# envoyproxy/ai-gateway

Hardware: AMD Instinct MI355X
Metric: req/sec (whole node) + p50 added latency, OpenAI chat/completions 4k-token body (higher is better)
Workload: dtype bf16; 1 GPU; model=aigw standalone: OpenAI /v1/chat/completions -> mock upstream (examples/basic), global_batch=128, seq_len=4096, parallelism=dp1, front=fast, cpu_affinity=numa node 0 (128 cpus)

## Files before the change

csrc/aigw_fast_module.cpp:

```cpp

#include <pybind11/pybind11.h>
#include <pybind11/stl.h>

#include <cstdint>
#include <stdexcept>
#include <string>
#include <vector>

#include "fastpath.h"

namespace py = pybind11;
using namespace aigw_fast;

namespace aigw_fast {

GpuAdmissionDirect* admission_create(const long long* htab_keys,
                                     const int32_t* htab_rank, int htab_n,
                                     size_t max_bytes, int max_req, int device);
bool admission_count(GpuAdmissionDirect* a, const char* bytes, size_t n,
                     const int64_t* offsets, int n_req, int32_t* counts_out);
void admission_destroy(GpuAdmissionDirect* a);
bool admission_init_cache(GpuAdmissionDirect* a, const uint16_t* emb, int vocab,
                          const uint16_t* proj, int dim, long long capacity,
                          float threshold, int pending_cap, bool fp8);
// ... 243 lines not shown
          "swap_routes",
          [](FastServer& s, py::list route_specs) {
            std::vector<FastRoute> routes;
            for (auto item : route_specs) {
              py::dict rd = item.cast<py::dict>();
              FastRoute r;
              r.name = rd["name"].cast<std::string>();
              r.model_match = rd["model_match"].cast<std::string>();
              r.retries = rd["retries"].cast<int>();
              r.has_costs = rd["has_costs"].cast<bool>();
              r.eligible = rd["eligible"].cast<bool>();
              for (auto b : rd["backends"].cast<py::list>()) {
                py::dict d = b.cast<py::dict>();
                FastBackend be;
                be.name = d["name"].cast<std::string>();
                be.host = d["host"].cast<std::string>();
                be.port = d["port"].cast<uint16_t>();
                if (d.contains("bearer")) be.bearer = d["bearer"].cast<std::string>();
                if (d.contains("api_key_file"))
                  be.api_key_file = d["api_key_file"].cast<std::string>();
                if (d.contains("model_override"))
                  be.model_override = d["model_override"].cast<std::string>();
                if (d.contains("weight")) be.weight = d["weight"].cast<double>();
                if (d.contains("priority")) be.priority = d["priority"].cast<int>();
                if (d.contains("timeout_s")) be.timeout_s = d["timeout_s"].cast<double>();
                if (d.contains("azure")) be.azure = d["azure"].cast<bool>();
                if (d.contains("azure_api_version"))
                  be.azure_api_version = d["azure_api_version"].cast<std::string>();
                r.backends.push_back(std::move(be));
              }
              routes.push_back(std::move(r));
            }
            s.swap_routes(std::move(routes));
          },
          "hot-swap the route table (in-flight requests keep the old one)")
      .def("drain", &FastServer::drain, py::arg("drain_s"),
           py::call_guard<py::gil_scoped_release>())
      .def("enable_gpu", &FastServer::enable_gpu, py::arg("socket_path"),
           py::arg("window_us") = 100, py::arg("max_batch") = 256)
      .def(
          "enable_gpu_direct",
          [](FastServer& s, py::buffer htab_keys, py::buffer htab_rank,
             int max_batch, size_t max_batch_bytes, int max_req, int device) {
            py::buffer_info ki = htab_keys.request();
            py::buffer_info ri = htab_rank.request();
            if (ki.itemsize != 8 || ri.itemsize != 4)
              throw std::runtime_error(
                  "htab_keys must be int64, htab_rank int32");
            if (ki.size != ri.size)
              throw std::runtime_error("htab arrays must have equal length");
            s.enable_gpu_direct(static_cast<const long long*>(ki.ptr),
                                static_cast<const int32_t*>(ri.ptr),
                                (int)ki.size, max_batch, max_batch_bytes,
                                max_req, device);
          },
          py::arg("htab_keys"), py::arg("htab_rank"),
          py::arg("max_batch") = 1024,
          py::arg("max_batch_bytes") = (size_t)48 * 1024 * 1024,
          py::arg("max_req") = 4096, py::arg("device") = 0)
      .def(
          "enable_gpu_direct_cache",
          [](FastServer& s, py::buffer emb, py::buffer proj, int dim,
             long long capacity, float threshold, bool fp8) {
            py::buffer_info ei = emb.request();
            py::buffer_info pi = proj.request();
            if (ei.itemsize != 2 || pi.itemsize != 2)
              throw std::runtime_error("emb/proj must be bf16 (uint16 view)");
            int vocab = (int)(ei.size / dim);
            if ((long long)vocab * dim != ei.size || pi.size != (long long)dim * dim)
              throw std::runtime_error("emb/proj shape mismatch");
            if (!s.enable_gpu_direct_cache(
                    static_cast<const uint16_t*>(ei.ptr), vocab,
                    static_cast<const uint16_t*>(pi.ptr), dim, capacity,
                    threshold, fp8))
              throw std::runtime_error("native cache init failed");
          },
          py::arg("emb"), py::arg("proj"), py::arg("dim") = 384,
          py::arg("capacity") = 65536, py::arg("threshold") = 0.92,
          py::arg("fp8") = false)
      .def("start", &FastServer::start, py::arg("host"), py::arg("port"),
           py::call_guard<py::gil_scoped_release>())
      .def("stop", &FastServer::stop, py::call_guard<py::gil_scoped_release>())
      .def("gpu_direct_stats", &FastServer::gpu_direct_stats)
      .def("rl_collect_deltas", &FastServer::rl_collect_deltas)
      .def("rl_apply_remote", &FastServer::rl_apply_remote)
      .def("rl_local_spent", &FastServer::rl_local_spent)
      .def("stats", [](const FastServer& s) {
        const ServerStats& st = s.stats();
        py::dict d;
        d["requests"] = st.requests.load();
        d["responses_2xx"] = st.responses_2xx.load();
        d["responses_4xx"] = st.responses_4xx.load();
        d["responses_5xx"] = st.responses_5xx.load();
        d["local_429"] = st.local_429.load();
        d["fallback"] = st.fallback.load();
        d["retries"] = st.retries.load();
        d["gpu_tokens"] = st.gpu_tokens.load();
        d["cache_hits"] = st.cache_hits.load();
        d["cache_misses"] = st.cache_misses.load();
        d["input_tokens"] = st.input_tokens.load();
        d["output_tokens"] = st.output_tokens.load();
        d["total_tokens"] = st.total_tokens.load();
        d["bytes_in"] = st.bytes_in.load();
        d["bytes_out"] = st.bytes_out.load();
        d["active_connections"] = st.active_connections.load();
        py::list hist;
        for (int i = 0; i < 32; ++i) hist.append(st.latency_us_log2[i].load());
        d["latency_us_log2"] = hist;
        return d;
      });
}
```

csrc/fastpath.cpp:

```cpp

#include "fastpath.h"

#include <arpa/inet.h>
#include <errno.h>
#include <fcntl.h>
#include <netdb.h>
#include <netinet/in.h>
#include <netinet/tcp.h>
#include <string.h>
#include <sys/socket.h>
#include <sys/time.h>
#include <sys/types.h>
#include <sys/un.h>
#include <unistd.h>

#include <algorithm>
#include <chrono>
#include <cmath>
#include <random>

#include "msgpack_mini.h"
#include "native_core.h"

namespace aigw_fast {
// ... 51 lines not shown
  struct msghdr msg;
  memset(&msg, 0, sizeof(msg));
  msg.msg_iov = iov;
  msg.msg_iovlen = 2;
  while (sent < total) {
    ssize_t w = ::sendmsg(fd, &msg, MSG_NOSIGNAL);
    if (w < 0) {
      if (errno == EINTR) continue;
      return false;
    }
    sent += (size_t)w;
    size_t skip = (size_t)w;
    while (msg.msg_iovlen > 0 && skip >= msg.msg_iov[0].iov_len) {
      skip -= msg.msg_iov[0].iov_len;
      ++msg.msg_iov;
      --msg.msg_iovlen;
    }
    if (msg.msg_iovlen > 0) {
      msg.msg_iov[0].iov_base = (char*)msg.msg_iov[0].iov_base + skip;
      msg.msg_iov[0].iov_len -= skip;
    }
  }
  return true;
}

ssize_t read_some(int fd, char* p, size_t cap) {
  for (;;) {
    ssize_t r = ::recv(fd, p, cap, 0);
    if (r < 0 && errno == EINTR) continue;
    return r;
  }
}

int tcp_connect(const std::string& host, uint16_t port, double timeout_s) {
  struct sockaddr_in addr;
  memset(&addr, 0, sizeof(addr));
  addr.sin_family = AF_INET;
  addr.sin_port = htons(port);
  if (inet_pton(AF_INET, host.c_str(), &addr.sin_addr) != 1) {
    struct addrinfo hints, *res = nullptr;
    memset(&hints, 0, sizeof(hints));
    hints.ai_family = AF_INET;
    hints.ai_socktype = SOCK_STREAM;
    if (getaddrinfo(host.c_str(), nullptr, &hints, &res) != 0 || !res) return -1;
    addr.sin_addr = ((struct sockaddr_in*)res->ai_addr)->sin_addr;
    freeaddrinfo(res);
  }
  int fd = ::socket(AF_INET, SOCK_STREAM, 0);
  if (fd < 0) return -1;
  set_timeout(fd, timeout_s);
  if (::connect(fd, (struct sockaddr*)&addr, sizeof(addr)) != 0) {
    ::close(fd);
    return -1;
  }
  set_nodelay(fd);
  return fd;
}

std::string lower(std::string s) {
  for (auto& c : s) c = (char)tolower((unsigned char)c);
  return s;
}

struct Header {
  std::string name;
  std::string value;
};

struct HttpHead {
  std::string method, path;
  int status = 0;
  std::vector<Header> headers;
  size_t head_len = 0;

  const std::string* get(const char* name) const {
    for (const auto& h : headers)
      if (h.name == name) return &h.value;
    return nullptr;
  }
};

constexpr size_t kMaxHead = 64 * 1024;
constexpr size_t kMaxBody = 64 * 1024 * 1024;

bool parse_head(const std::string& buf, size_t head_end, bool is_request, HttpHead* out) {
  out->head_len = head_end + 4;
  size_t line_end = buf.find("\r\n");
  if (line_end == std::string::npos || line_end > head_end) return false;
  const std::string first = buf.substr(0, line_end);
  if (is_request) {
    size_t sp1 = first.find(' ');
    if (sp1 == std::string::npos) return false;
    size_t sp2 = first.find(' ', sp1 + 1);
    if (sp2 == std::string::npos) return false;
    out->method = first.substr(0, sp1);
    out->path = first.substr(sp1 + 1, sp2 - sp1 - 1);
  } else {
    if (first.compare(0, 7, "HTTP/1.") != 0) return false;
    size_t sp = first.find(' ');
    if (sp == std::string::npos) return false;
    out->status = atoi(first.c_str() + sp + 1);
  }
  size_t pos = line_end + 2;
  while (pos < head_end) {
    size_t eol = buf.find("\r\n", pos);
    if (eol == std::string::npos || eol > head_end) eol = head_end;
    size_t colon = buf.find(':', pos);
    if (colon != std::string::npos && colon < eol) {
      Header h;
      h.name = lower(buf.substr(pos, colon - pos));
      size_t vs = colon + 1;
      while (vs < eol && (buf[vs] == ' ' || buf[vs] == '\t')) ++vs;
      size_t ve = eol;
      while (ve > vs && (buf[ve - 1] == ' ' || buf[ve - 1] == '\t')) --ve;
      while (!h.name.empty() && (h.name.back() == ' ' || h.name.back() == '\t'))
        h.name.pop_back();
      h.value = buf.substr(vs, ve - vs);
      out->headers.push_back(std::move(h));
    }
    pos = eol + 2;
  }
  return true;
}


enum class Framing { kLength, kChunked, kClose, kNone };

Framing response_framing(const HttpHead& h, int64_t* length) {
  const std::string* te = h.get("transfer-encoding");
  if (te && lower(*te).find("chunked") != std::string::npos) return Framing::kChunked;
  if (h.status == 204 || h.status == 304 || (h.status >= 100 && h.status < 200)) {
    *length = 0;
    return Framing::kLength;
  }
  const std::string* cl = h.get("content-length");
  if (cl) {
    *length = atoll(cl->c_str());
    return Framing::kLength;
  }
  return Framing::kClose;
}

class ChunkedParser {
 public:
  bool done() const { return state_ == State::kDone; }
  bool error() const { return state_ == State::kError; }

  template <class F>
  void feed(const char* p, size_t n, F&& payload) {
    size_t i = 0;
    while (i < n && state_ != State::kDone && state_ != State::kError) {
      switch (state_) {
        case State::kSize: {
          char c = p[i++];
          line_.push_back(c);
          if (line_.size() > 256) { state_ = State::kError; break; }
          if (c == '\n') {
            size_t semi = line_.find(';');
            std::string hex = line_.substr(0, semi);
            remaining_ = strtoll(hex.c_str(), nullptr, 16);
            line_.clear();
            if (remaining_ < 0) state_ = State::kError;
            else if (remaining_ == 0) state_ = State::kTrailer;
            else state_ = State::kData;
          }
          break;
// ... 307 lines not shown
    std::vector<std::shared_ptr<Waiter>> all;
    {
      std::lock_guard<std::mutex> lk(qmu_);
      all.insert(all.end(), q_waiters_.begin(), q_waiters_.end());
      q_waiters_.clear();
      q_texts_.clear();
    }
    {
      std::lock_guard<std::mutex> lk(pmu_);
      for (auto& kv : pending_)
        all.insert(all.end(), kv.second.begin(), kv.second.end());
      pending_.clear();
    }
    for (auto& w : all) {
      std::lock_guard<std::mutex> lk(w->m);
      w->done = true;
      w->cv.notify_all();
    }
  }

  int fd_ = -1;
  int window_us_ = 100;
  int max_batch_ = 256;
  std::atomic<bool> stopping_{false};
  std::atomic<uint64_t> next_id_{1};
  std::mutex qmu_;
  std::condition_variable qcv_;
  std::vector<std::string> q_texts_;
  std::vector<std::shared_ptr<GpuAdmissionClient::Waiter>> q_waiters_;
  std::mutex pmu_;
  std::map<uint64_t, std::vector<std::shared_ptr<Waiter>>> pending_;
  std::thread batcher_, reader_;
};



GpuAdmissionDirect* admission_create(const long long* htab_keys,
                                     const int32_t* htab_rank, int htab_n,
                                     size_t max_bytes, int max_req, int device);
bool admission_count(GpuAdmissionDirect* a, const char* bytes, size_t n,
                     const int64_t* offsets, int n_req, int32_t* counts_out);
void admission_destroy(GpuAdmissionDirect* a);
bool admission_init_cache(GpuAdmissionDirect* a, const uint16_t* emb, int vocab,
                          const uint16_t* proj, int dim, long long capacity,
                          float threshold, int pending_cap, bool fp8);
bool admission_count_lookup(GpuAdmissionDirect* a, const char* bytes, size_t n,
                            const int64_t* offsets, int n_req,
                            int32_t* counts_out, const int32_t* pending_slots,
                            int32_t* rows_out, float* scores_out);
long long admission_cache_insert(GpuAdmissionDirect* a, int pending_slot);
bool admission_submit(GpuAdmissionDirect* a, int set, const char* bytes,
                      size_t n, const int64_t* offsets, int n_req,
                      const int32_t* pending_slots);
bool admission_wait(GpuAdmissionDirect* a, int set, int n_req,
                    int32_t* counts_out, int32_t* rows_out, float* scores_out);
char* admission_staging(GpuAdmissionDirect* a, int set);

class DirectGpuBatcher {
 public:
  bool start(const long long* htab_keys, const int32_t* htab_rank, int htab_n,
             int max_batch, size_t max_bytes, int max_req, int device) {
    adm_ = admission_create(htab_keys, htab_rank, htab_n, max_bytes, max_req,
                            device);
    if (adm_ == nullptr) return false;
    max_batch_ = std::min(max_batch, max_req);
    max_bytes_ = max_bytes;
    worker_ = std::thread([this] { loop(); });
    return true;
  }

  void stop() {
    stopping_ = true;
    {
      std::lock_guard<std::mutex> lk(mu_);
      cv_.notify_all();
    }
    if (worker_.joinable()) worker_.join();
    if (adm_ != nullptr) admission_destroy(adm_), adm_ = nullptr;
    fail_all();
  }

  ~DirectGpuBatcher() { stop(); }

  int64_t count_text(const std::string& text) {
    CacheLookup cl = count_lookup_text(text);
    cache_release_slot(cl.slot);
    return cl.tokens;
  }

  struct Waiter2 {
    std::mutex m;
    std::condition_variable cv;
    bool done = false;
    int64_t count = 0;
    int32_t row = -1;
    float score = 0.f;
    int32_t slot = -1;
  };

  struct CacheLookup {
    int64_t tokens = 0;
    int32_t row = -1;
    float score = 0.f;
    int32_t slot = -1;
  };

  std::shared_ptr<Waiter2> enqueue(const std::string& text) {
    if (stopping_) return nullptr;
    auto w = std::make_shared<Waiter2>();
    {
      std::lock_guard<std::mutex> lk(mu_);
      q_texts_.push_back(text);
      q_waiters_.push_back(w);
      cv_.notify_one();
    }
    return w;
  }

  CacheLookup collect(const std::shared_ptr<Waiter2>& w) {
    CacheLookup out;
    if (w == nullptr) return out;
    std::unique_lock<std::mutex> lk(w->m);
    w->cv.wait_for(lk, std::chrono::seconds(30), [&] { return w->done; });
    out.tokens = w->count;
    out.row = w->row;
    out.score = w->score;
    out.slot = w->slot;
    return out;
  }

  CacheLookup count_lookup_text(const std::string& text) {
    return collect(enqueue(text));
  }

  bool init_cache(const uint16_t* emb, int vocab, const uint16_t* proj,
                  int dim, long long capacity, float threshold, bool fp8) {
    if (adm_ == nullptr) return false;
    const int pending_cap = 4096;
    if (!admission_init_cache(adm_, emb, vocab, proj, dim, capacity, threshold,
                              pending_cap, fp8))
      return false;
    {
      std::lock_guard<std::mutex> lk(slot_mu_);
      free_slots_.resize(pending_cap);
      for (int i = 0; i < pending_cap; ++i) free_slots_[i] = pending_cap - 1 - i;
    }
    cache_on_ = true;
    return true;
  }

  bool cache_on() const { return cache_on_; }

  long long cache_insert_slot(int slot) {
    long long row;
    {
      std::lock_guard<std::mutex> lk(insert_mu_);
      row = admission_cache_insert(adm_, slot);
    }
    cache_release_slot(slot);
    return row;
  }

  void cache_release_slot(int slot) {
    if (slot < 0) return;
    std::lock_guard<std::mutex> lk(slot_mu_);
    free_slots_.push_back(slot);
  }


 private:
  struct InFlight {
    std::vector<std::shared_ptr<Waiter2>> waiters;
    std::vector<int32_t> slots;
    int64_t t0 = 0;
    bool valid = false;
  };

  void finish_set(int s) {
    InFlight& fl = inflight_[s];
    if (!fl.valid) return;
    int n = (int)fl.waiters.size();
    std::vector<int32_t> counts((size_t)n, 0);
    std::vector<int32_t> rows((size_t)n, -1);
    std::vector<float> scores((size_t)n, 0.f);
    bool want_cache = cache_on_.load();
    int64_t w0 = now_us();
    if (!admission_wait(adm_, s, n, counts.data(),
                        want_cache ? rows.data() : nullptr,
                        want_cache ? scores.data() : nullptr))
      stats_errors++;
    int64_t w1 = now_us();
    stats_wait_us += (uint64_t)(w1 - w0);
    int64_t bt = w1 - fl.t0;
    stats_batches++;
    stats_texts += (uint64_t)n;
    stats_time_us += (uint64_t)bt;
    uint64_t prev = stats_max_us.load();
    while ((uint64_t)bt > prev &&
           !stats_max_us.compare_exchange_weak(prev, (uint64_t)bt)) {}
    for (int i = 0; i < n; ++i) {
      auto& w = fl.waiters[i];
      std::lock_guard<std::mutex> lk(w->m);
      w->count = counts[i];
      w->row = rows[i];
      w->score = scores[i];
      w->slot = fl.slots[i];
      w->done = true;
      w->cv.notify_all();
    }
    stats_fulfill_us += (uint64_t)(now_us() - w1);
    fl.waiters.clear();
    fl.slots.clear();
    fl.valid = false;
  }

  void loop() {
    std::vector<int64_t> offs;
    int next_set = 0;
    while (!stopping_) {
      std::vector<std::string> texts;
      std::vector<std::shared_ptr<Waiter2>> waiters;
      {
        std::unique_lock<std::mutex> lk(mu_);
        if (q_texts_.empty()) {
          int other = 1 - next_set;
          if (inflight_[other].valid) {
            lk.unlock();
            finish_set(other);
            continue;
          }
          cv_.wait(lk, [&] { return stopping_ || !q_texts_.empty(); });
          if (stopping_) break;
        }
        size_t take = 0, bytes = 0;
        while (take < q_texts_.size() && (int)take < max_batch_ &&
               bytes + q_texts_[take].size() <= max_bytes_)
          bytes += q_texts_[take++].size();
        if (take == 0) take = 1;
        texts.assign(q_texts_.begin(), q_texts_.begin() + take);
        waiters.assign(q_waiters_.begin(), q_waiters_.begin() + take);
        q_texts_.erase(q_texts_.begin(), q_texts_.begin() + take);
        q_waiters_.erase(q_waiters_.begin(), q_waiters_.begin() + take);
      }
      finish_set(next_set);
      int64_t p0 = now_us();
      char* stage = admission_staging(adm_, next_set);
      size_t used = 0;
      offs.clear();
      for (auto& t : texts) {
        offs.push_back((int64_t)used);
        size_t room = max_bytes_ - used;
        size_t take_n = std::min(t.size(), room);
        memcpy(stage + used, t.data(), take_n);
        used += take_n;
      }
      size_t nt = texts.size();
      std::vector<int32_t> slots((size_t)nt, -1);
      if (cache_on_) {
        std::lock_guard<std::mutex> lk(slot_mu_);
        for (size_t i = 0; i < nt && !free_slots_.empty(); ++i) {
          slots[i] = free_slots_.back();
          free_slots_.pop_back();
        }
      }
      stats_pack_us += (uint64_t)(now_us() - p0);
      int64_t s0 = now_us();
      bool ok = used > 0 &&
                admission_submit(adm_, next_set, nullptr, used,
                                 offs.data(), (int)nt,
                                 cache_on_ ? slots.data() : nullptr);
      stats_submit_us += (uint64_t)(now_us() - s0);
      if (!ok) {
        if (used > 0) stats_errors++;
        for (size_t i = 0; i < nt; ++i) {
          auto& w = waiters[i];
          std::lock_guard<std::mutex> lk(w->m);
          w->slot = slots[i];
          w->done = true;
          w->cv.notify_all();
        }
        continue;
      }
      InFlight& fl = inflight_[next_set];
      fl.waiters = std::move(waiters);
      fl.slots = std::move(slots);
      fl.t0 = now_us();
      fl.valid = true;
      finish_set(1 - next_set);
      next_set ^= 1;
    }
    finish_set(0);
    finish_set(1);
  }

  void fail_all() {
    std::vector<std::shared_ptr<Waiter2>> all;
    {
      std::lock_guard<std::mutex> lk(mu_);
      all = std::move(q_waiters_);
      q_waiters_.clear();
      q_texts_.clear();
    }
    for (auto& w : all) {
      std::lock_guard<std::mutex> lk(w->m);
      w->done = true;
      w->cv.notify_all();
    }
  }

  GpuAdmissionDirect* adm_ = nullptr;
  std::atomic<bool> cache_on_{false};
  std::mutex slot_mu_;
  std::vector<int32_t> free_slots_;
  std::mutex insert_mu_;

 public:
  std::atomic<uint64_t> stats_batches{0};
  std::atomic<uint64_t> stats_texts{0};
  std::atomic<uint64_t> stats_time_us{0};
  std::atomic<uint64_t> stats_max_us{0};
  std::atomic<uint64_t> stats_errors{0};
  std::atomic<uint64_t> stats_pack_us{0};
  std::atomic<uint64_t> stats_submit_us{0};
  std::atomic<uint64_t> stats_wait_us{0};
  std::atomic<uint64_t> stats_fulfill_us{0};

 private:
  int max_batch_ = 1024;
  size_t max_bytes_ = 0;
  std::atomic<bool> stopping_{false};
  std::mutex mu_;
  std::condition_variable cv_;
  std::vector<std::string> q_texts_;
  std::vector<std::shared_ptr<Waiter2>> q_waiters_;
  InFlight inflight_[2];
  std::thread worker_;
};



namespace {

bool banned_upstream_header(const std::string& name) {
  static const char* kBanned[] = {
      "host", "content-length", "content-type", "connection", "keep-alive",
      "proxy-authenticate", "proxy-authorization", "te", "trailer",
      "transfer-encoding", "upgrade", "expect", "accept-encoding",
      "authorization"};
  for (const char* b : kBanned)
    if (name == b) return true;
  if (name.compare(0, 8, "x-ai-eg-") == 0) return true;
  if (name.compare(0, 7, "x-aigw-") == 0) return true;
  return false;
}

}

class ConnHandler {
 public:
  ConnHandler(FastServer* srv, int fd) : srv_(srv), fd_(fd) {}

  void run() {
    std::string buf;
    char tmp[65536];
    for (;;) {
      size_t head_end;
      for (;;) {
        head_end = buf.find("\r\n\r\n");
        if (head_end != std::string::npos) break;
        if (buf.size() > kMaxHead) return;
        ssize_t r = read_some(fd_, tmp, sizeof(tmp));
        if (r <= 0) return;
        srv_->stats_.bytes_in += (uint64_t)r;
        buf.append(tmp, (size_t)r);
      }
      HttpHead req;
      if (!parse_head(buf, head_end, true, &req)) {
        simple_reply(400, "invalid_request_error", "malformed request", true);
        return;
      }
      int64_t clen = 0;
      bool te = false, dup_conflict = false;
      {
        const std::string* seen = nullptr;
        for (const auto& h : req.headers) {
          if (h.name == "transfer-encoding") te = true;
          if (h.name == "content-length") {
            if (seen && *seen != h.value) dup_conflict = true;
            seen = &h.value;
          }
        }
        if (seen) clen = atoll(seen->c_str());
      }
      if (te) {
        simple_reply(501, "invalid_request_error", "transfer-encoding not supported", true);
        return;
      }
      if (dup_conflict || clen < 0 || (size_t)clen > kMaxBody) {
        simple_reply(400, "invalid_request_error", "bad content-length", true);
        return;
      }
      while (buf.size() < req.head_len + (size_t)clen) {
        ssize_t r = read_some(fd_, tmp, sizeof(tmp));
        if (r <= 0) return;
        srv_->stats_.bytes_in += (uint64_t)r;
        buf.append(tmp, (size_t)r);
      }
      std::string body = buf.substr(req.head_len, (size_t)clen);
      buf.erase(0, req.head_len + (size_t)clen);

      bool keep = handle_request(req, body);
      if (!keep) return;
    }
  }

 private:
  bool handle_request(const HttpHead& req, const std::string& body) {
    srv_->stats_.requests++;
    if (req.method == "GET" && req.path == "/health") {
      return raw_reply(200, "application/json",
                       "{\"status\":\"ok\",\"front\":\"fast\"}");
    }
    bool hot = req.method == "POST" &&
               (req.path == "/v1/chat/completions" || req.path == "/v1/completions" ||
                req.path == "/v1/embeddings");
    if (!hot) return fallback(req, body);

    int64_t t0 = now_us();
    aigw_core::Scan sc{body.data(), body.data() + body.size()};
    sc.base = body.data();
    bool ok = sc.parse_value(0, "", true) && sc.ok;
    if (ok) {
      sc.ws();
      ok = sc.p == sc.end;
    }
    if (!ok) {
      srv_->stats_.responses_4xx++;
      return simple_reply(400, "invalid_request_error",
                          "invalid request body: malformed JSON", false);
    }
    if (sc.model.empty()) {
      srv_->stats_.responses_4xx++;
      return simple_reply(400, "invalid_request_error",
                          "missing required field 'model'", false);
    }
    std::shared_ptr<const std::vector<FastRoute>> table =
        std::atomic_load(&srv_->routes_);
    const FastRoute* route = nullptr;
    for (const auto& r : *table) {
      if (r.catch_all || r.model_match == sc.model) {
        route = &r;
        break;
      }
    }
    if (!route) {
      srv_->stats_.responses_4xx++;
      return simple_reply(404, "model_not_found",
                          "no route matched model " + sc.model, false);
    }
    if (!route->eligible) return fallback(req, body);
    bool stream = sc.stream == 1 && req.path != "/v1/embeddings";

    double retry_after = 0;
    std::string rule_name;
    if (!srv_->rl_check(&retry_after, &rule_name)) {
      srv_->stats_.local_429++;
      srv_->stats_.responses_4xx++;
      std::string extra = "retry-after: " + std::to_string((int)retry_after + 1) + "\r\n";
      return simple_reply(429, "rate_limit_exceeded", "token budget exhausted",
                          false, extra);
    }

    int64_t gpu_tokens = 0;
    int32_t cache_slot = -1;
    uint64_t cache_fp = 0;
    pending_count_.reset();
    bool cache_eligible = srv_->gpu_direct_ != nullptr &&
                          srv_->gpu_direct_->cache_on() && !stream &&
                          req.path == "/v1/chat/completions" &&
                          !sc.text.empty();
    if (cache_eligible) {
      cache_fp = 1469598103934665603ull;
      auto fnv = [&](const char* p, size_t n) {
        for (size_t i = 0; i < n; ++i) {
          cache_fp ^= (unsigned char)p[i];
          cache_fp *= 1099511628211ull;
        }
      };
      fnv(route->name.data(), route->name.size());
      fnv(sc.model.data(), sc.model.size());
      const std::string* auth_h = req.get("authorization");
      if (auth_h) fnv(auth_h->data(), auth_h->size());
      if (sc.msgs_ve > sc.msgs_vs && sc.msgs_ve <= body.size()) {
        fnv(body.data(), sc.msgs_vs);
        fnv(body.data() + sc.msgs_ve, body.size() - sc.msgs_ve);
      } else {
        fnv(body.data(), body.size());
      }
      auto cl = srv_->gpu_direct_->count_lookup_text(sc.text);
      gpu_tokens = cl.tokens;
      srv_->stats_.gpu_tokens += (uint64_t)gpu_tokens;
      cache_slot = cl.slot;
      if (cl.row >= 0) {
        std::string hit;
        {
          std::lock_guard<std::mutex> lk(srv_->cache_mu_);
          if ((size_t)cl.row < srv_->cache_values_.size())
            hit = srv_->cache_values_[cl.row];
        }
        if (hit.size() > 9 &&
            memcmp(hit.data(), &cache_fp, 8) == 0 && hit[8] == 'U') {
          srv_->gpu_direct_->cache_release_slot(cache_slot);
          srv_->stats_.cache_hits++;
          srv_->stats_.responses_2xx++;
          record_latency(t0);
          std::string h =
              "HTTP/1.1 200 X\r\ncontent-type: application/json\r\n"
              "x-aigw-cache: hit\r\ncontent-length: " +
              std::to_string(hit.size() - 9) + "\r\n\r\n";
          std::string bodyv = hit.substr(9);
          srv_->stats_.bytes_out += h.size() + bodyv.size();
          return write_two(fd_, h, bodyv);
        }
      }
      srv_->stats_.cache_misses++;
    } else if (srv_->gpu_enabled() && req.path == "/v1/chat/completions" &&
               !sc.text.empty()) {
      if (srv_->gpu_direct_ != nullptr && stream) {
        pending_count_ = srv_->gpu_direct_->enqueue(sc.text);
      } else {
        gpu_tokens = srv_->gpu_count(sc.text);
        srv_->stats_.gpu_tokens += (uint64_t)gpu_tokens;
      }
    }

    std::vector<const FastBackend*> order;
    if (route->backends.size() == 1)
      order.push_back(&route->backends[0]);
    else
      order = attempt_order(*route);
    int attempts_left = std::min((int)order.size(), route->retries + 1);
    bool first = true;
    for (const FastBackend* be : order) {
      if (attempts_left-- <= 0) break;
      if (!first) srv_->stats_.retries++;
      first = false;
      int outcome = try_backend(req, body, sc, *route, *be, stream, gpu_tokens,
                                t0, cache_slot, cache_fp);
      if (outcome == 0) return true;
      if (outcome == 2) return false;
    }
    if (cache_slot >= 0) srv_->gpu_direct_->cache_release_slot(cache_slot);
    pending_count_.reset();
    srv_->stats_.responses_5xx++;
    return simple_reply(503, "upstream_error", "no healthy upstream", false);
  }

  std::vector<const FastBackend*> attempt_order(const FastRoute& route) {
    std::vector<const FastBackend*> order;
    order.reserve(route.backends.size());
    static thread_local std::mt19937_64 rng{std::random_device{}()};
    std::uniform_real_distribution<double> uni(1e-12, 1.0);
    size_t i = 0;
    while (i < route.backends.size()) {
      size_t j = i;
      while (j < route.backends.size() &&
             route.backends[j].priority == route.backends[i].priority)
        ++j;
      std::vector<std::pair<double, const FastBackend*>> keyed;
      for (size_t k = i; k < j; ++k) {
        double w = std::max(route.backends[k].weight, 1e-9);
        keyed.push_back({-std::pow(uni(rng), 1.0 / w), &route.backends[k]});
      }
      std::sort(keyed.begin(), keyed.end(),
                [](const auto& a, const auto& b) { return a.first < b.first; });
      for (auto& kv : keyed) order.push_back(kv.second);
      i = j;
    }
    return order;
  }

  int try_backend(const HttpHead& req, const std::string& body,
                  const aigw_core::Scan& sc, const FastRoute& route,
                  const FastBackend& be, bool stream, int64_t gpu_tokens,
                  int64_t t0, int32_t cache_slot = -1, uint64_t cache_fp = 0) {
    std::string out_body;
    const std::string* send_body = &body;
    if (!be.model_override.empty() && sc.model_ve > sc.model_vs) {
      out_body = splice_model(body, sc.model_vs, sc.model_ve, be.model_override);
      send_body = &out_body;
    }
    if (stream && route.has_costs) {
      if (send_body == &body) out_body = body, send_body = &out_body;
      splice_include_usage(&out_body);
    }

    std::string head;
    head.reserve(512 + req.head_len);
    head += "POST ";
    if (be.azure) {
      const std::string& model_eff =
          be.model_override.empty() ? sc.model : be.model_override;
      const char* suffix = req.path == "/v1/embeddings" ? "embeddings"
                           : req.path == "/v1/completions"
                               ? "completions"
                               : "chat/completions";
      head += "/openai/deployments/" + model_eff + "/" + suffix +
              "?api-version=" +
              (be.azure_api_version.empty() ? "2025-01-01-preview"
                                            : be.azure_api_version);
    } else {
      head += req.path;
    }
    head += " HTTP/1.1\r\nhost: ";
// ... 279 lines not shown
      if (head_end != std::string::npos) break;
      ssize_t r = read_some(ufd, tmp, sizeof(tmp));
      if (r <= 0 || rbuf.size() > kMaxHead) {
        ::close(ufd);
        return simple_reply(502, "upstream_error", "fallback read failed", false);
      }
      rbuf.append(tmp, (size_t)r);
    }
    HttpHead resp;
    if (!parse_head(rbuf, head_end, false, &resp)) {
      ::close(ufd);
      return simple_reply(502, "upstream_error", "fallback bad response", false);
    }
    rbuf.erase(0, resp.head_len);
    int64_t length = -1;
    Framing fr = response_framing(resp, &length);
    bool up_close = false;
    {
      const std::string* c = resp.get("connection");
      if (c && lower(*c).find("close") != std::string::npos) up_close = true;
    }
    std::string chead = "HTTP/1.1 " + std::to_string(resp.status) + " X\r\n";
    for (const auto& h : resp.headers) {
      if (h.name == "connection" || h.name == "keep-alive") continue;
      chead += h.name + ": " + h.value + "\r\n";
    }
    bool client_close = fr == Framing::kClose;
    if (client_close) chead += "connection: close\r\n";
    chead += "\r\n";
    if (!write_all(fd_, chead)) {
      ::close(ufd);
      return false;
    }
    srv_->stats_.bytes_out += chead.size();
    ChunkedParser cp;
    int64_t remaining = length;
    bool done = (fr == Framing::kLength && length == 0), up_err = false;
    auto pump = [&](const char* p, size_t n) -> bool {
      if (n == 0) return true;
      if (fr == Framing::kChunked) {
        cp.feed(p, n, [](const char*, size_t) {});
        if (cp.error()) up_err = true;
        if (cp.done()) done = true;
      } else if (fr == Framing::kLength) {
        remaining -= (int64_t)n;
        if (remaining <= 0) done = true;
      }
      srv_->stats_.bytes_out += n;
      return write_all(fd_, p, n);
    };
    if (!pump(rbuf.data(), rbuf.size())) {
      ::close(ufd);
      return false;
    }
    rbuf.clear();
    while (!done && !up_err) {
      ssize_t r = read_some(ufd, tmp, sizeof(tmp));
      if (r < 0) {
        up_err = true;
        break;
      }
      if (r == 0) {
        if (fr == Framing::kClose) done = true;
        else up_err = true;
        break;
      }
      if (!pump(tmp, (size_t)r)) {
        ::close(ufd);
        return false;
      }
    }
    if (resp.status < 400) srv_->stats_.responses_2xx++;
    else if (resp.status < 500) srv_->stats_.responses_4xx++;
    else srv_->stats_.responses_5xx++;
    if (up_err || fr == Framing::kClose || up_close)
      ::close(ufd);
    else
      srv_->pool_->release(srv_->fallback_host_, srv_->fallback_port_, ufd, true);
    return !client_close && !up_err;
  }

  int64_t resolve_pending_count() {
    if (pending_count_ == nullptr) return 0;
    auto cl = srv_->gpu_direct_->collect(pending_count_);
    pending_count_.reset();
    srv_->gpu_direct_->cache_release_slot(cl.slot);
    srv_->stats_.gpu_tokens += (uint64_t)cl.tokens;
    return cl.tokens;
  }

  void finish_usage(Usage& u, int64_t gpu_tokens) {
    if (pending_count_ != nullptr) {
      int64_t t = resolve_pending_count();
      if (gpu_tokens == 0) gpu_tokens = t;
    }
    if (u.total == 0 && gpu_tokens > 0) {
      u.input = gpu_tokens;
      u.total = gpu_tokens + u.output;
    }
    srv_->stats_.input_tokens += (uint64_t)u.input;
    srv_->stats_.output_tokens += (uint64_t)u.output;
    srv_->stats_.total_tokens += (uint64_t)u.total;
    srv_->rl_charge(u);
  }

  void record_latency(int64_t t0) {
    int64_t us = now_us() - t0;
    if (us < 1) us = 1;
    int b = 63 - __builtin_clzll((uint64_t)us);
    if (b > 31) b = 31;
    srv_->stats_.latency_us_log2[b]++;
  }

  bool raw_reply(int status, const char* ctype, const std::string& body) {
    std::string head = "HTTP/1.1 " + std::to_string(status) + " X\r\ncontent-type: " +
                       ctype + "\r\ncontent-length: " + std::to_string(body.size()) +
                       "\r\n\r\n";
    srv_->stats_.bytes_out += head.size() + body.size();
    return write_two(fd_, head, body);
  }

  bool simple_reply(int status, const char* type, const std::string& msg,
                    bool close_after, const std::string& extra_headers = "") {
    std::string body = "{\"type\":\"error\",\"error\":{\"type\":\"";
    body += type;
    body += "\",\"code\":\"";
    body += std::to_string(status);
    body += "\",\"message\":\"";
    for (char c : msg) {
      if (c == '"' || c == '\\') body.push_back('\\');
      if ((unsigned char)c >= 0x20) body.push_back(c);
    }
    body += "\"}}";
    std::string head = "HTTP/1.1 " + std::to_string(status) +
                       " X\r\ncontent-type: application/json\r\ncontent-length: " +
                       std::to_string(body.size()) + "\r\n" + extra_headers;
    if (close_after) head += "connection: close\r\n";
    head += "\r\n";
    srv_->stats_.bytes_out += head.size() + body.size();
    bool ok = write_two(fd_, head, body);
    return ok && !close_after;
  }

  FastServer* srv_;
  int fd_;
  std::shared_ptr<DirectGpuBatcher::Waiter2> pending_count_;

  friend class FastServer;
};



int FastMock::start(const std::string& host, const std::string& response) {
    response_ = response;
    listen_fd_ = ::socket(AF_INET, SOCK_STREAM, 0);
    if (listen_fd_ < 0) throw std::runtime_error("mock socket() failed");
    int one = 1;
    setsockopt(listen_fd_, SOL_SOCKET, SO_REUSEADDR, &one, sizeof(one));
    struct sockaddr_in addr;
    memset(&addr, 0, sizeof(addr));
    addr.sin_family = AF_INET;
    addr.sin_port = 0;
    inet_pton(AF_INET, host.c_str(), &addr.sin_addr);
    if (::bind(listen_fd_, (struct sockaddr*)&addr, sizeof(addr)) != 0 ||
        ::listen(listen_fd_, 4096) != 0)
      throw std::runtime_error("mock bind/listen failed");
    socklen_t alen = sizeof(addr);
    getsockname(listen_fd_, (struct sockaddr*)&addr, &alen);
    acceptor_ = std::thread([this] {
      for (;;) {
        int fd = ::accept(listen_fd_, nullptr, nullptr);
        if (fd < 0) return;
        set_nodelay(fd);
        set_timeout(fd, 300.0);
        std::thread([this, fd] { serve(fd); }).detach();
      }
    });
    return ntohs(addr.sin_port);
}

void FastMock::stop() {
    if (listen_fd_ >= 0) {
      ::shutdown(listen_fd_, SHUT_RDWR);
      ::close(listen_fd_);
      listen_fd_ = -1;
    }
    if (acceptor_.joinable()) acceptor_.join();
}

uint64_t FastMock::requests() const { return served_.load(); }

void FastMock::serve(int fd) {
    std::string buf;
    char tmp[65536];
    for (;;) {
      size_t head_end;
      for (;;) {
        head_end = buf.find("\r\n\r\n");
        if (head_end != std::string::npos) break;
        ssize_t r = read_some(fd, tmp, sizeof(tmp));
        if (r <= 0) { ::close(fd); return; }
        buf.append(tmp, (size_t)r);
      }
      int64_t clen = 0;
      {
        size_t p = buf.find("content-length:");
        if (p == std::string::npos) p = buf.find("Content-Length:");
        if (p != std::string::npos && p < head_end)
          clen = atoll(buf.c_str() + p + 15);
      }
      while (buf.size() < head_end + 4 + (size_t)clen) {
        ssize_t r = read_some(fd, tmp, sizeof(tmp));
        if (r <= 0) { ::close(fd); return; }
        buf.append(tmp, (size_t)r);
      }
      buf.erase(0, head_end + 4 + (size_t)clen);
      if (!write_all(fd, response_)) { ::close(fd); return; }
      served_++;
    }
}

LoadResult run_load_pool(const std::string& host, uint16_t port,
                         const std::string& path,
                         const std::vector<std::string>& bodies,
                         int connections, int per_conn, bool capture_last) {
  std::vector<std::string> reqs;
  reqs.reserve(bodies.size());
  for (const auto& body : bodies)
    reqs.push_back("POST " + path + " HTTP/1.1\r\nhost: bench\r\n"
// ... 81 lines not shown
  for (auto& t : threads) t.join();
  LoadResult out;
  out.elapsed_s = (double)(now_us() - t0) / 1e6;
  out.completed = completed.load();
  out.errors = errors.load();
  out.last_bodies = std::move(last);
  std::vector<int64_t> all;
  for (auto& v : lat) all.insert(all.end(), v.begin(), v.end());
  if (!all.empty()) {
    std::sort(all.begin(), all.end());
    out.p50_ms = (double)all[all.size() / 2] / 1e3;
    out.p99_ms = (double)all[std::min(all.size() - 1,
                                      (size_t)((double)all.size() * 0.99))] / 1e3;
  }
  return out;
}

LoadResult run_load(const std::string& host, uint16_t port,
                    const std::string& path, const std::string& body,
                    int connections, int per_conn) {
  return run_load_pool(host, port, path, {body}, connections, per_conn);
}


FastServer::FastServer() : pool_(new UpstreamPool) {}

FastServer::~FastServer() { stop(); }

static void normalize_route(FastRoute& r) {
  std::stable_sort(r.backends.begin(), r.backends.end(),
                   [](const FastBackend& a, const FastBackend& b) {
                     return a.priority < b.priority;
                   });
  if (r.model_match.empty()) r.catch_all = true;
}

void FastServer::add_route(FastRoute r) {
  normalize_route(r);
  auto next = std::make_shared<std::vector<FastRoute>>(*routes_);
  next->push_back(std::move(r));
  routes_ = std::move(next);
}

void FastServer::swap_routes(std::vector<FastRoute> routes) {
  for (auto& r : routes) normalize_route(r);
  std::atomic_store(&routes_,
                    std::shared_ptr<const std::vector<FastRoute>>(
                        std::make_shared<const std::vector<FastRoute>>(
                            std::move(routes))));
}

void FastServer::add_rate_rule(const RateRule& r) {
  auto rs = std::make_unique<RuleState>();
  rs->rule = r;
  rs->window_start_ms = now_ms();
  rules_.push_back(std::move(rs));
}

void FastServer::set_fallback(const std::string& host, uint16_t port) {
  fallback_host_ = host;
  fallback_port_ = port;
}

void FastServer::enable_gpu(const std::string& socket_path, int window_us,
                            int max_batch) {
  auto client = std::make_unique<GpuAdmissionClient>();
  if (!client->start(socket_path, window_us, max_batch)) {
    throw std::runtime_error("cannot connect GPU admission service at " + socket_path);
  }
  gpu_.push_back(std::move(client));
}

std::vector<uint64_t> FastServer::gpu_direct_stats() const {
  if (gpu_direct_ == nullptr) return {0, 0, 0, 0, 0, 0, 0, 0, 0};
  return {gpu_direct_->stats_batches.load(), gpu_direct_->stats_texts.load(),
          gpu_direct_->stats_time_us.load(), gpu_direct_->stats_max_us.load(),
          gpu_direct_->stats_errors.load(),
          gpu_direct_->stats_pack_us.load(),
          gpu_direct_->stats_submit_us.load(),
          gpu_direct_->stats_wait_us.load(),
          gpu_direct_->stats_fulfill_us.load()};
}

bool FastServer::gpu_enabled() const {
  return gpu_direct_ != nullptr || !gpu_.empty();
}

int64_t FastServer::gpu_count(const std::string& text) {
  if (gpu_direct_ != nullptr) return gpu_direct_->count_text(text);
  size_t i = (size_t)(gpu_rr_.fetch_add(1, std::memory_order_relaxed) % gpu_.size());
  return gpu_[i]->count_text(text);
}

bool FastServer::enable_gpu_direct_cache(const uint16_t* emb, int vocab,
                                         const uint16_t* proj, int dim,
                                         long long capacity, float threshold,
                                         bool fp8) {
  if (gpu_direct_ == nullptr) return false;
  if (!gpu_direct_->init_cache(emb, vocab, proj, dim, capacity, threshold, fp8))
    return false;
  cache_values_.assign((size_t)capacity, std::string());
  return true;
}

void FastServer::enable_gpu_direct(const long long* htab_keys,
                                   const int32_t* htab_rank, int htab_n,
                                   int max_batch, size_t max_batch_bytes,
                                   int max_req, int device) {
  auto b = std::make_unique<DirectGpuBatcher>();
  if (!b->start(htab_keys, htab_rank, htab_n, max_batch, max_batch_bytes,
                max_req, device))
    throw std::runtime_error(
        "direct GPU admission init failed (no device visible?)");
  gpu_direct_ = std::move(b);
}

int FastServer::start(const std::string& host, uint16_t port) {
  listen_fd_ = ::socket(AF_INET, SOCK_STREAM, 0);
  if (listen_fd_ < 0) throw std::runtime_error("socket() failed");
  int one = 1;
  setsockopt(listen_fd_, SOL_SOCKET, SO_REUSEADDR, &one, sizeof(one));
  struct sockaddr_in addr;
  memset(&addr, 0, sizeof(addr));
  addr.sin_family = AF_INET;
  addr.sin_port = htons(port);
  if (inet_pton(AF_INET, host.c_str(), &addr.sin_addr) != 1)
    addr.sin_addr.s_addr = INADDR_ANY;
  if (::bind(listen_fd_, (struct sockaddr*)&addr, sizeof(addr)) != 0) {
    ::close(listen_fd_);
    listen_fd_ = -1;
    throw std::runtime_error("bind failed: " + std::string(strerror(errno)));
  }
  if (::listen(listen_fd_, 4096) != 0) {
    ::close(listen_fd_);
    listen_fd_ = -1;
    throw std::runtime_error("listen failed");
  }
  socklen_t alen = sizeof(addr);
  getsockname(listen_fd_, (struct sockaddr*)&addr, &alen);
  acceptor_ = std::thread([this] { accept_loop(); });
  return ntohs(addr.sin_port);
}

void FastServer::accept_loop() {
  for (;;) {
    int fd = ::accept(listen_fd_, nullptr, nullptr);
    if (fd < 0) {
      if (errno == EINTR) continue;
      return;
    }
    if (stopping_) {
      ::close(fd);
      return;
    }
    set_nodelay(fd);
    set_timeout(fd, 300.0);
    {
      std::lock_guard<std::mutex> lk(conn_mu_);
      if (conn_fds_.size() >= 8192) {
        ::close(fd);
        continue;
      }
      conn_fds_.insert(fd);
    }
    stats_.active_connections++;
    std::thread([this, fd] {
// ... 130 lines not shown
```

csrc/fastpath.h:

```cpp
#pragma once

#include <atomic>
#include <condition_variable>
#include <cstdint>
#include <map>
#include <memory>
#include <mutex>
#include <set>
#include <string>
#include <thread>
#include <vector>

namespace aigw_fast {

struct FastBackend {
  std::string name;
  std::string host;
  uint16_t port = 0;
  std::string bearer;
  std::string api_key_file;
  std::string model_override;
  bool azure = false;
  std::string azure_api_version;
  double weight = 1.0;
  int priority = 0;
  double timeout_s = 60.0;
};

struct FastRoute {
  std::string name;
  std::string model_match;
  bool catch_all = false;
  int retries = 1;
  bool has_costs = false;
  bool eligible = true;
  std::vector<FastBackend> backends;
};

struct RateRule {
  std::string name;
  int64_t limit = 0;
  double window_s = 60.0;
  int metadata_key = 0;
};

struct Usage {
  int64_t input = 0, output = 0, total = 0;
};

struct ServerStats {
  std::atomic<uint64_t> requests{0};
  std::atomic<uint64_t> responses_2xx{0};
  std::atomic<uint64_t> responses_4xx{0};
  std::atomic<uint64_t> responses_5xx{0};
  std::atomic<uint64_t> local_429{0};
  std::atomic<uint64_t> fallback{0};
  std::atomic<uint64_t> retries{0};
  std::atomic<uint64_t> gpu_tokens{0};
  std::atomic<uint64_t> cache_hits{0};
  std::atomic<uint64_t> cache_misses{0};
  std::atomic<uint64_t> input_tokens{0};
  std::atomic<uint64_t> output_tokens{0};
  std::atomic<uint64_t> total_tokens{0};
  std::atomic<uint64_t> bytes_in{0};
  std::atomic<uint64_t> bytes_out{0};
  std::atomic<uint64_t> active_connections{0};
  std::atomic<uint64_t> latency_us_log2[32] = {};
};

class GpuAdmissionClient;
class GpuAdmissionDirect;
class DirectGpuBatcher;
class UpstreamPool;

class FastServer {
 public:
  FastServer();
  ~FastServer();

  void add_route(FastRoute r);
  void swap_routes(std::vector<FastRoute> routes);
  void add_rate_rule(const RateRule& r);
  void set_fallback(const std::string& host, uint16_t port);
  void enable_gpu(const std::string& socket_path, int window_us, int max_batch);
  void enable_gpu_direct(const long long* htab_keys, const int32_t* htab_rank,
                         int htab_n, int max_batch, size_t max_batch_bytes,
                         int max_req, int device);
  bool enable_gpu_direct_cache(const uint16_t* emb, int vocab,
                               const uint16_t* proj, int dim,
                               long long capacity, float threshold,
                               bool fp8);

  int start(const std::string& host, uint16_t port);
  int drain(double drain_s);
  void stop();

  const ServerStats& stats() const { return stats_; }
  std::vector<uint64_t> gpu_direct_stats() const;
  std::vector<int64_t> rl_collect_deltas();
  void rl_apply_remote(const std::vector<int64_t>& others_spend);
  std::vector<int64_t> rl_local_spent() const;

  std::string resolve_bearer(const FastBackend& be);

 private:
  friend class ConnHandler;
  struct FileCredState {
    int64_t checked_ms = 0;
    std::string value;
  };
  struct RuleState {
    RateRule rule;
    std::atomic<int64_t> window_start_ms{0};
    std::atomic<int64_t> local_spent{0};
    std::atomic<int64_t> remote_spent{0};
    std::atomic<int64_t> pending_delta{0};
  };

  void accept_loop();
  void handle_connection(int fd);
  bool rl_check(double* retry_after_s, std::string* rule_name);
  void rl_charge(const Usage& u);
  void rl_roll(RuleState& rs, int64_t now_ms);

  std::shared_ptr<const std::vector<FastRoute>> routes_ =
      std::make_shared<const std::vector<FastRoute>>();
  std::vector<std::unique_ptr<RuleState>> rules_;
  std::string fallback_host_;
  uint16_t fallback_port_ = 0;
  std::vector<std::unique_ptr<GpuAdmissionClient>> gpu_;
  std::unique_ptr<DirectGpuBatcher> gpu_direct_;
  std::atomic<uint64_t> gpu_rr_{0};
  int64_t gpu_count(const std::string& text);
  bool gpu_enabled() const;
  std::unique_ptr<UpstreamPool> pool_;
  ServerStats stats_;

  int listen_fd_ = -1;
  std::atomic<bool> stopping_{false};
  std::thread acceptor_;
  std::mutex conn_mu_;
  std::set<int> conn_fds_;
  std::mutex cred_mu_;
  std::map<std::string, FileCredState> file_creds_;
  std::mutex cache_mu_;
  std::vector<std::string> cache_values_;
};


class FastMock {
 public:
  int start(const std::string& host, const std::string& response);
  void stop();
  uint64_t requests() const;
  ~FastMock() { stop(); }

 private:
  void serve(int fd);
  std::string response_;
  int listen_fd_ = -1;
  std::thread acceptor_;
  std::atomic<uint64_t> served_{0};
};

struct LoadResult {
  double elapsed_s = 0;
  uint64_t completed = 0;
  uint64_t errors = 0;
  double p50_ms = 0, p99_ms = 0;
  std::vector<std::string> last_bodies;
};

LoadResult run_load(const std::string& host, uint16_t port,
                    const std::string& path, const std::string& body,
                    int connections, int per_conn);
LoadResult run_load_pool(const std::string& host, uint16_t port,
                         const std::string& path,
                         const std::vector<std::string>& bodies,
                         int connections, int per_conn,
                         bool capture_last = false);

// ... 2 lines not shown
```

csrc/native_core.h:

```cpp
#pragma once

#include <cstddef>
#include <cstring>
#include <string>
#include <utility>
#include <vector>

namespace aigw_core {

struct Scan {
  const char* p;
  const char* end;
  std::string model;
  int stream = 0;
  std::string text;
  bool ok = true;
  const char* base = nullptr;
  size_t model_vs = 0, model_ve = 0;
  size_t msgs_vs = 0, msgs_ve = 0;

  void ws() {
    while (p < end && (*p == ' ' || *p == '\t' || *p == '\n' || *p == '\r')) ++p;
  }

  bool parse_string(std::string* collect) {
    if (p >= end || *p != '"') return fail();
    ++p;
    while (p < end) {
      const char* seg = p;
      while (p < end && *p != '"' && *p != '\\') ++p;
      if (collect && p != seg) collect->append(seg, p - seg);
      if (p >= end) return fail();
      unsigned char c = *p;
      if (c == '"') {
        ++p;
        return true;
      }
      if (c == '\\') {
        if (p + 1 >= end) return fail();
        char e = p[1];
        p += 2;
        if (!collect) {
          switch (e) {
            case '"': case '\\': case '/': case 'b': case 'f':
            case 'n': case 'r': case 't':
              break;
            case 'u': {
              if (p + 4 > end) return fail();
              for (int i = 0; i < 4; ++i) {
                char h = p[i];
                if (!((h >= '0' && h <= '9') || (h >= 'a' && h <= 'f') ||
                      (h >= 'A' && h <= 'F')))
                  return fail();
              }
              p += 4;
              break;
            }
            default:
              return fail();
          }
          continue;
        }
        switch (e) {
          case '"': collect->push_back('"'); break;
          case '\\': collect->push_back('\\'); break;
          case '/': collect->push_back('/'); break;
          case 'b': collect->push_back('\b'); break;
          case 'f': collect->push_back('\f'); break;
          case 'n': collect->push_back('\n'); break;
          case 'r': collect->push_back('\r'); break;
          case 't': collect->push_back('\t'); break;
          case 'u': {
            if (p + 4 > end) return fail();
            unsigned v = 0;
            for (int i = 0; i < 4; ++i) {
              char h = p[i];
              v <<= 4;
              if (h >= '0' && h <= '9') v |= h - '0';
              else if (h >= 'a' && h <= 'f') v |= h - 'a' + 10;
              else if (h >= 'A' && h <= 'F') v |= h - 'A' + 10;
              else return fail();
            }
            p += 4;
            if (v >= 0xD800 && v <= 0xDBFF && p + 6 <= end && p[0] == '\\' &&
                p[1] == 'u') {
              unsigned lo = 0;
              bool okp = true;
              for (int i = 0; i < 4; ++i) {
                char h = p[2 + i];
                lo <<= 4;
                if (h >= '0' && h <= '9') lo |= h - '0';
                else if (h >= 'a' && h <= 'f') lo |= h - 'a' + 10;
                else if (h >= 'A' && h <= 'F') lo |= h - 'A' + 10;
                else { okp = false; break; }
              }
              if (okp && lo >= 0xDC00 && lo <= 0xDFFF) {
                v = 0x10000 + ((v - 0xD800) << 10) + (lo - 0xDC00);
                p += 6;
              }
            }
            if (v < 0x80) collect->push_back((char)v);
            else if (v < 0x800) {
              collect->push_back((char)(0xC0 | (v >> 6)));
              collect->push_back((char)(0x80 | (v & 0x3F)));
            } else if (v < 0x10000) {
              collect->push_back((char)(0xE0 | (v >> 12)));
              collect->push_back((char)(0x80 | ((v >> 6) & 0x3F)));
              collect->push_back((char)(0x80 | (v & 0x3F)));
            } else {
              collect->push_back((char)(0xF0 | (v >> 18)));
              collect->push_back((char)(0x80 | ((v >> 12) & 0x3F)));
              collect->push_back((char)(0x80 | ((v >> 6) & 0x3F)));
              collect->push_back((char)(0x80 | (v & 0x3F)));
// ... 184 lines not shown
```

Baseline: 190,500 req/s.

## Cut per-request string copies in gateway fast path and SIMD-scan JSON strings

Request texts are now moved into the batcher waiter instead of copied into a separate queue. The worker swaps the whole queue when it fits in one batch, and each connection reuses its body and text buffers across requests, reading the body straight into place. JSON string scanning now uses SSE2 to find quotes and backslashes 16 bytes at a time, and waiters are notified outside their mutex. The aim is to remove allocation, copy and lock overhead on 4k-token bodies, at the cost of extra buffer-ownership plumbing and a new take-time stat.

```diff
diff --git a/csrc/aigw_fast_module.cpp b/csrc/aigw_fast_module.cpp
--- a/csrc/aigw_fast_module.cpp
+++ b/csrc/aigw_fast_module.cpp
@@ -349,6 +349,7 @@
            py::call_guard<py::gil_scoped_release>())
       .def("stop", &FastServer::stop, py::call_guard<py::gil_scoped_release>())
       .def("gpu_direct_stats", &FastServer::gpu_direct_stats)
+      .def("gpu_direct_take_us", &FastServer::gpu_direct_take_us)
       .def("rl_collect_deltas", &FastServer::rl_collect_deltas)
       .def("rl_apply_remote", &FastServer::rl_apply_remote)
       .def("rl_local_spent", &FastServer::rl_local_spent)
diff --git a/csrc/fastpath.cpp b/csrc/fastpath.cpp
--- a/csrc/fastpath.cpp
+++ b/csrc/fastpath.cpp
@@ -157,6 +157,7 @@
 
 constexpr size_t kMaxHead = 64 * 1024;
 constexpr size_t kMaxBody = 64 * 1024 * 1024;
+constexpr size_t kKeepBuf = 1024 * 1024;
 
 bool parse_head(const std::string& buf, size_t head_end, bool is_request, HttpHead* out) {
   out->head_len = head_end + 4;
@@ -630,15 +631,20 @@
 
   ~DirectGpuBatcher() { stop(); }
 
-  int64_t count_text(const std::string& text) {
-    CacheLookup cl = count_lookup_text(text);
+  int64_t count_text(std::string&& text, std::string* reclaim = nullptr) {
+    CacheLookup cl = count_lookup_text(std::move(text), reclaim);
     cache_release_slot(cl.slot);
     return cl.tokens;
+  }
+
+  int64_t count_text(const std::string& text) {
+    return count_text(std::string(text));
   }
 
   struct Waiter2 {
     std::mutex m;
     std::condition_variable cv;
+    std::string text;
     bool done = false;
     int64_t count = 0;
     int32_t row = -1;
@@ -653,23 +659,34 @@
     int32_t slot = -1;
   };
 
-  std::shared_ptr<Waiter2> enqueue(const std::string& text) {
+  std::shared_ptr<Waiter2> enqueue(std::string&& text) {
     if (stopping_) return nullptr;
     auto w = std::make_shared<Waiter2>();
+    w->text = std::move(text);
+    size_t n = w->text.size();
     {
       std::lock_guard<std::mutex> lk(mu_);
-      q_texts_.push_back(text);
-      q_waiters_.push_back(w);
+      q_.push_back(w);
+      q_bytes_ += n;
       cv_.notify_one();
     }
     return w;
   }
 
-  CacheLookup collect(const std::shared_ptr<Waiter2>& w) {
+  std::shared_ptr<Waiter2> enqueue(const std::string& text) {
+    return enqueue(std::string(text));
+  }
+
+  CacheLookup collect(const std::shared_ptr<Waiter2>& w,
+                      std::string* reclaim = nullptr) {
     CacheLookup out;
     if (w == nullptr) return out;
     std::unique_lock<std::mutex> lk(w->m);
     w->cv.wait_for(lk, std::chrono::seconds(30), [&] { return w->done; });
+    if (w->done && reclaim != nullptr) {
+      reclaim->swap(w->text);
+      reclaim->clear();
+    }
     out.tokens = w->count;
     out.row = w->row;
     out.score = w->score;
@@ -677,8 +694,13 @@
     return out;
   }
 
+  CacheLookup count_lookup_text(std::string&& text,
+                                std::string* reclaim = nullptr) {
+    return collect(enqueue(std::move(text)), reclaim);
+  }
+
   CacheLookup count_lookup_text(const std::string& text) {
-    return collect(enqueue(text));
+    return collect(enqueue(std::string(text)));
   }
 
   bool init_cache(const uint16_t* emb, int vocab, const uint16_t* proj,
@@ -748,12 +770,14 @@
            !stats_max_us.compare_exchange_weak(prev, (uint64_t)bt)) {}
     for (int i = 0; i < n; ++i) {
       auto& w = fl.waiters[i];
-      std::lock_guard<std::mutex> lk(w->m);
-      w->count = counts[i];
-      w->row = rows[i];
-      w->score = scores[i];
-      w->slot = fl.slots[i];
-      w->done = true;
+      {
+        std::lock_guard<std::mutex> lk(w->m);
+        w->count = counts[i];
+        w->row = rows[i];
+        w->score = scores[i];
+        w->slot = fl.slots[i];
+        w->done = true;
+      }
       w->cv.notify_all();
     }
     stats_fulfill_us += (uint64_t)(now_us() - w1);
@@ -765,44 +789,55 @@
   void loop() {
     std::vector<int64_t> offs;
     int next_set = 0;
+    std::vector<std::shared_ptr<Waiter2>> waiters;
     while (!stopping_) {
-      std::vector<std::string> texts;
-      std::vector<std::shared_ptr<Waiter2>> waiters;
+      int64_t k0 = now_us();
       {
         std::unique_lock<std::mutex> lk(mu_);
-        if (q_texts_.empty()) {
+        if (q_.empty()) {
           int other = 1 - next_set;
           if (inflight_[other].valid) {
             lk.unlock();
             finish_set(other);
             continue;
           }
-          cv_.wait(lk, [&] { return stopping_ || !q_texts_.empty(); });
+          cv_.wait(lk, [&] { return stopping_ || !q_.empty(); });
           if (stopping_) break;
+          k0 = now_us();
         }
-        size_t take = 0, bytes = 0;
-        while (take < q_texts_.size() && (int)take < max_batch_ &&
-               bytes + q_texts_[take].size() <= max_bytes_)
-          bytes += q_texts_[take++].size();
-        if (take == 0) take = 1;
-        texts.assign(q_texts_.begin(), q_texts_.begin() + take);
-        waiters.assign(q_waiters_.begin(), q_waiters_.begin() + take);
-        q_texts_.erase(q_texts_.begin(), q_texts_.begin() + take);
-        q_waiters_.erase(q_waiters_.begin(), q_waiters_.begin() + take);
-      }
+        if (q_.size() <= (size_t)max_batch_ && q_bytes_ <= max_bytes_) {
+          waiters.swap(q_);
+          q_bytes_ = 0;
+        } else {
+          size_t take = 0, bytes = 0;
+          while (take < q_.size() && (int)take < max_batch_ &&
+                 bytes + q_[take]->text.size() <= max_bytes_)
+            bytes += q_[take++]->text.size();
+          if (take == 0) {
+            take = 1;
+            bytes = q_[0]->text.size();
+          }
+          waiters.assign(std::make_move_iterator(q_.begin()),
+                         std::make_move_iterator(q_.begin() + take));
+          q_.erase(q_.begin(), q_.begin() + take);
+          q_bytes_ -= bytes;
+        }
+      }
+      stats_take_us += (uint64_t)(now_us() - k0);
       finish_set(next_set);
       int64_t p0 = now_us();
       char* stage = admission_staging(adm_, next_set);
       size_t used = 0;
       offs.clear();
-      for (auto& t : texts) {
+      for (auto& w : waiters) {
+        const std::string& t = w->text;
         offs.push_back((int64_t)used);
         size_t room = max_bytes_ - used;
         size_t take_n = std::min(t.size(), room);
         memcpy(stage + used, t.data(), take_n);
         used += take_n;
       }
-      size_t nt = texts.size();
+      size_t nt = waiters.size();
       std::vector<int32_t> slots((size_t)nt, -1);
       if (cache_on_) {
         std::lock_guard<std::mutex> lk(slot_mu_);
@@ -822,15 +857,18 @@
         if (used > 0) stats_errors++;
         for (size_t i = 0; i < nt; ++i) {
           auto& w = waiters[i];
-          std::lock_guard<std::mutex> lk(w->m);
-          w->slot = slots[i];
-          w->done = true;
+          {
+            std::lock_guard<std::mutex> lk(w->m);
+            w->slot = slots[i];
+            w->done = true;
+          }
           w->cv.notify_all();
         }
+        waiters.clear();
         continue;
       }
       InFlight& fl = inflight_[next_set];
-      fl.waiters = std::move(waiters);
+      fl.waiters.swap(waiters);
       fl.slots = std::move(slots);
       fl.t0 = now_us();
       fl.valid = true;
@@ -845,13 +883,15 @@
     std::vector<std::shared_ptr<Waiter2>> all;
     {
       std::lock_guard<std::mutex> lk(mu_);
-      all = std::move(q_waiters_);
-      q_waiters_.clear();
-      q_texts_.clear();
+      all = std::move(q_);
+      q_.clear();
+      q_bytes_ = 0;
     }
     for (auto& w : all) {
-      std::lock_guard<std::mutex> lk(w->m);
-      w->done = true;
+      {
+        std::lock_guard<std::mutex> lk(w->m);
+        w->done = true;
+      }
       w->cv.notify_all();
     }
   }
@@ -872,6 +912,7 @@
   std::atomic<uint64_t> stats_submit_us{0};
   std::atomic<uint64_t> stats_wait_us{0};
   std::atomic<uint64_t> stats_fulfill_us{0};
+  std::atomic<uint64_t> stats_take_us{0};
 
  private:
   int max_batch_ = 1024;
@@ -879,8 +920,8 @@
   std::atomic<bool> stopping_{false};
   std::mutex mu_;
   std::condition_variable cv_;
-  std::vector<std::string> q_texts_;
-  std::vector<std::shared_ptr<Waiter2>> q_waiters_;
+  std::vector<std::shared_ptr<Waiter2>> q_;
+  size_t q_bytes_ = 0;
   InFlight inflight_[2];
   std::thread worker_;
 };
@@ -910,6 +951,7 @@
 
   void run() {
     std::string buf;
+    std::string body;
     char tmp[65536];
     for (;;) {
       size_t head_end;
@@ -948,17 +990,27 @@
         simple_reply(400, "invalid_request_error", "bad content-length", true);
         return;
       }
-      while (buf.size() < req.head_len + (size_t)clen) {
-        ssize_t r = read_some(fd_, tmp, sizeof(tmp));
-        if (r <= 0) return;
-        srv_->stats_.bytes_in += (uint64_t)r;
-        buf.append(tmp, (size_t)r);
-      }
-      std::string body = buf.substr(req.head_len, (size_t)clen);
-      buf.erase(0, req.head_len + (size_t)clen);
+      const size_t need = (size_t)clen;
+      size_t have = std::min(buf.size() - req.head_len, need);
+      body.assign(buf.data() + req.head_len, have);
+      if (req.head_len + have == buf.size())
+        buf.clear();
+      else
+        buf.erase(0, req.head_len + have);
+      if (have < need) {
+        body.resize(need);
+        while (have < need) {
+          ssize_t r = read_some(fd_, &body[have], need - have);
+          if (r <= 0) return;
+          srv_->stats_.bytes_in += (uint64_t)r;
+          have += (size_t)r;
+        }
+      }
 
       bool keep = handle_request(req, body);
       if (!keep) return;
+      if (body.capacity() > kKeepBuf) std::string().swap(body);
+      if (text_buf_.capacity() > kKeepBuf) std::string().swap(text_buf_);
     }
   }
 
@@ -977,6 +1029,18 @@
     int64_t t0 = now_us();
     aigw_core::Scan sc{body.data(), body.data() + body.size()};
     sc.base = body.data();
+    text_buf_.clear();
+    sc.text.swap(text_buf_);
+    struct TextReturn {
+      std::string& from;
+      std::string& to;
+      ~TextReturn() {
+        if (from.capacity() > to.capacity()) {
+          to.swap(from);
+          to.clear();
+        }
+      }
+    } text_return{sc.text, text_buf_};
     bool ok = sc.parse_value(0, "", true) && sc.ok;
     if (ok) {
       sc.ws();
@@ -1045,7 +1109,8 @@
       } else {
         fnv(body.data(), body.size());
       }
-      auto cl = srv_->gpu_direct_->count_lookup_text(sc.text);
+      auto cl = srv_->gpu_direct_->count_lookup_text(std::move(sc.text),
+                                                     &text_buf_);
       gpu_tokens = cl.tokens;
       srv_->stats_.gpu_tokens += (uint64_t)gpu_tokens;
       cache_slot = cl.slot;
@@ -1075,9 +1140,12 @@
     } else if (srv_->gpu_enabled() && req.path == "/v1/chat/completions" &&
                !sc.text.empty()) {
       if (srv_->gpu_direct_ != nullptr && stream) {
-        pending_count_ = srv_->gpu_direct_->enqueue(sc.text);
+        pending_count_ = srv_->gpu_direct_->enqueue(std::move(sc.text));
       } else {
-        gpu_tokens = srv_->gpu_count(sc.text);
+        gpu_tokens = srv_->gpu_direct_ != nullptr
+                         ? srv_->gpu_direct_->count_text(std::move(sc.text),
+                                                         &text_buf_)
+                         : srv_->gpu_count(sc.text);
         srv_->stats_.gpu_tokens += (uint64_t)gpu_tokens;
       }
     }
@@ -1523,7 +1591,7 @@
 
   int64_t resolve_pending_count() {
     if (pending_count_ == nullptr) return 0;
-    auto cl = srv_->gpu_direct_->collect(pending_count_);
+    auto cl = srv_->gpu_direct_->collect(pending_count_, &text_buf_);
     pending_count_.reset();
     srv_->gpu_direct_->cache_release_slot(cl.slot);
     srv_->stats_.gpu_tokens += (uint64_t)cl.tokens;
@@ -1586,6 +1654,7 @@
   FastServer* srv_;
   int fd_;
   std::shared_ptr<DirectGpuBatcher::Waiter2> pending_count_;
+  std::string text_buf_;
 
   friend class FastServer;
 };
@@ -1833,6 +1902,10 @@
           gpu_direct_->stats_fulfill_us.load()};
 }
 
+uint64_t FastServer::gpu_direct_take_us() const {
+  return gpu_direct_ == nullptr ? 0 : gpu_direct_->stats_take_us.load();
+}
+
 bool FastServer::gpu_enabled() const {
   return gpu_direct_ != nullptr || !gpu_.empty();
 }
diff --git a/csrc/fastpath.h b/csrc/fastpath.h
--- a/csrc/fastpath.h
+++ b/csrc/fastpath.h
@@ -97,6 +97,7 @@
 
   const ServerStats& stats() const { return stats_; }
   std::vector<uint64_t> gpu_direct_stats() const;
+  uint64_t gpu_direct_take_us() const;
   std::vector<int64_t> rl_collect_deltas();
   void rl_apply_remote(const std::vector<int64_t>& others_spend);
   std::vector<int64_t> rl_local_spent() const;
diff --git a/csrc/native_core.h b/csrc/native_core.h
--- a/csrc/native_core.h
+++ b/csrc/native_core.h
@@ -5,6 +5,10 @@
 #include <string>
 #include <utility>
 #include <vector>
+
+#if defined(__SSE2__)
+#include <emmintrin.h>
+#endif
 
 namespace aigw_core {
 
@@ -18,9 +22,30 @@
   const char* base = nullptr;
   size_t model_vs = 0, model_ve = 0;
   size_t msgs_vs = 0, msgs_ve = 0;
+  bool simd = true;
 
   void ws() {
     while (p < end && (*p == ' ' || *p == '\t' || *p == '\n' || *p == '\r')) ++p;
+  }
+
+  void skip_plain() {
+#if defined(__SSE2__)
+    if (simd) {
+      const __m128i q = _mm_set1_epi8('"');
+      const __m128i b = _mm_set1_epi8('\\');
+      while (end - p >= 16) {
+        __m128i v = _mm_loadu_si128(reinterpret_cast<const __m128i*>(p));
+        unsigned m = (unsigned)_mm_movemask_epi8(
+            _mm_or_si128(_mm_cmpeq_epi8(v, q), _mm_cmpeq_epi8(v, b)));
+        if (m) {
+          p += __builtin_ctz(m);
+          return;
+        }
+        p += 16;
+      }
+    }
+#endif
+    while (p < end && *p != '"' && *p != '\\') ++p;
   }
 
   bool parse_string(std::string* collect) {
@@ -28,7 +53,7 @@
     ++p;
     while (p < end) {
       const char* seg = p;
-      while (p < end && *p != '"' && *p != '\\') ++p;
+      skip_plain();
       if (collect && p != seg) collect->append(seg, p - seg);
       if (p >= end) return fail();
       unsigned char c = *p;
```

Measured after the change: 219,500 req/s, median of 6. +15.2%, better.
